# weihaoysgs/ssvio

Hardware: AMD Instinct MI355X
Metric: stereo frames/s (ORB extract + row-band match + triangulate + one local BA per frame) on 1241x376 (higher is better)
Workload: dtype u8 (front-end) + f64 (BA)

## Files before the change

include/ssx_test_hooks.h:

```cpp
#ifndef SSX_TEST_HOOKS_H
#define SSX_TEST_HOOKS_H
#include "ssx.h"

#ifdef __cplusplus
extern "C" {
#endif

SSX_API int32_t ssx_ba_window_selftest(uint32_t seed, int32_t steps);
SSX_API int32_t ssx_ba_window_debug_rewrites(const ssx_ba_window* win);

SSX_API int64_t ssx_debug_kernel_dynamic_lds(const char* kernel);
SSX_API void ssx_debug_set_dense_slabs(int32_t mode);

SSX_API void ssx_debug_set_trial_finish(int32_t mode);

SSX_API double ssx_ba_debug_prepare_seconds(const ssx_ba_problem* prob, int32_t reps);

SSX_API int32_t ssx_ba_debug_upload_format(const ssx_ba_problem* prob);

SSX_API uint64_t ssx_ba_debug_prepare_digest(const ssx_ba_problem* prob, int32_t threads);

typedef struct ssx_orb_plan_info {
  int32_t status, n_buffers;
  uint64_t digest[3];
  uint64_t arena_bytes, buf_off[32], buf_bytes[32];
  int32_t nlevels, out_cap;
  int32_t lvl_rows[8], lvl_cols[8], feat[8], lvl_cell0[9], gauss_tile0[9];
  char error[256];
} ssx_orb_plan_info;
SSX_API ssx_status ssx_orb_debug_plan(int32_t rows, int32_t cols, int32_t images, const ssx_orb_params* prm, int32_t has_mask,
                                      int32_t detect_only, int32_t unchecked, ssx_orb_plan_info* out);


SSX_API ssx_status ssx_ba_linearize(ssx_ctx* ctx, const ssx_ba_problem* prob, double huber_delta, int32_t jac_mode,
                            double* Hpp, double* bp, double* Hll, double* bl, double* Hpl, double* err,
                            double* chi2);

SSX_API ssx_status ssx_orb_stage_level(ssx_ctx* ctx, int32_t image, int32_t level, int32_t blurred,
                                       uint8_t* out, int32_t out_cap, int32_t* rows, int32_t* cols);
SSX_API ssx_status ssx_orb_stage_candidates(ssx_ctx* ctx, int32_t image, int32_t level, int32_t cap,
                                            ssx_keypoint* out, int32_t* n);

SSX_API ssx_status ssx_orb_debug_octree(ssx_ctx* ctx, int32_t rows, int32_t cols, int32_t images, const ssx_orb_params* prm,
                                        int32_t detect_only, int32_t n, const int32_t* image, const int32_t* level, const int32_t* x,
                                        const int32_t* y, const int32_t* response, int32_t* lvl_ncand, int32_t* sel_count,
                                        uint32_t* sel, int32_t* status);

SSX_API ssx_status ssx_lk_stage_level(ssx_ctx* ctx, int32_t which, int32_t level, uint8_t* out, int32_t out_cap,
                                      int32_t* rows, int32_t* cols);
SSX_API ssx_status ssx_lk_stage_deriv(ssx_ctx* ctx, int32_t level, int16_t* out, int32_t out_cap, int32_t* rows,
                                      int32_t* cols);

enum { SSX_LK_STAGED = 0, SSX_LK_ARENA = 1, SSX_LK_EACH = 2, SSX_LK_IN_PLACE = 3 };
enum { SSX_LK_K_PYRAMID = 0, SSX_LK_K_PAD_LEVEL0 = 1, SSX_LK_K_PYR_DOWN = 2, SSX_LK_K_SCHARR = 3, SSX_LK_K_TRACK = 4 };
enum { SSX_LK_SPANS = 7, SSX_LK_MAX_LAUNCHES = 32, SSX_LK_MAX_INFO_JOBS = 256 };
typedef struct ssx_lk_call_info {
  int32_t status;
  char error[256];
  int32_t levels, win, pad, rows[8], cols[8], pitch[8];
  uint64_t off[8], doff[8], pyr_bytes, deriv_words;
  int32_t fused_ok, use_fused, scharr_now, intake;
  uint64_t span_off[7], span_bytes[7], in_bytes, host_end, io_bytes, arena_bytes;
  int32_t n_launches, n_jobs;
  struct { int32_t kernel, grid[3], which, level; } launch[32];
  uint8_t slot_flags[256], job_roles[256];
} ssx_lk_call_info;
typedef struct ssx_lk_job_facts {
  int32_t slot, fresh, n, prev_stride, next_stride, reserved;
  int64_t next_off;
} ssx_lk_job_facts;
enum { SSX_LK_FACT_NEXT0_IS_HOST = 1, SSX_LK_FACT_SEVERAL_ALLOCATIONS = 2 };
SSX_API ssx_status ssx_lk_debug_plan(int32_t rows, int32_t cols, int32_t win, int32_t max_level, const int32_t* planned_key, int32_t n_jobs,
                                     const ssx_lk_job_facts* jobs, const uint8_t* slot_flags, int32_t images_on_device, int32_t call_facts,
                                     ssx_lk_call_info* out);
SSX_API ssx_status ssx_lk_debug_intake(ssx_ctx* ctx, int32_t n_jobs, const ssx_lk_job* jobs, int32_t rows, int32_t cols, const ssx_lk_params* prm,
                                       int32_t images_on_device, int32_t* intake, int32_t* arena_arithmetic);
SSX_API ssx_status ssx_lk_debug_last_call(ssx_ctx* ctx, ssx_lk_call_info* out);

SSX_API ssx_status ssx_pose_only_debug_trace(ssx_ctx* ctx, int32_t n, const ssx_pose_only_job* jobs, int32_t warmup, double* it_chi2,
                                             double* it_lambda, int32_t* it_trials, int32_t* round_rec);

enum { SSX_PO_SPANS = 6, SSX_PO_MAX_INFO_JOBS = 16, SSX_PNP_SPANS = 11 };
typedef struct ssx_po_plan_info {
  int32_t n_jobs, n_blocks, n_launches, reserved;
  struct { int32_t cls, block; uint64_t span_off[6], span_bytes[6]; } job[16];
  struct { uint64_t bytes, sent, ret_off, ret_bytes, desc_off, desc_bytes, trace_off, trace_bytes; } block[16];
  struct { int32_t cls, grid, block, first_desc; } launch[16];
} ssx_po_plan_info;
typedef struct ssx_pnp_plan_info {
  uint64_t span_off[11], span_bytes[11], bytes, sent, ret_off, ret_bytes;
  int32_t refine_cls, reserved;
} ssx_pnp_plan_info;
SSX_API ssx_status ssx_po_debug_plan(int32_t n, const int32_t* M, int32_t traced, ssx_po_plan_info* out, int32_t pnp_M, int32_t pnp_H,
                                     int32_t pnp_tap, ssx_pnp_plan_info* pnp_out);

SSX_API ssx_status ssx_pnp_debug_samples(ssx_ctx* ctx, uint32_t seed, int32_t M, int32_t H, int32_t* triples_out);
SSX_API ssx_status ssx_pnp_debug_counts(ssx_ctx* ctx, const double* K4, int32_t M, const double* xyz, const double* uv,
                                        int32_t max_iters, double reproj_px, uint32_t seed, int32_t* counts_out);
SSX_API ssx_status ssx_pnp_debug_p3p(ssx_ctx* ctx, const double* K4, int32_t n, const double* xyz, const double* uv, int32_t* valid_out,
                                     double* R_out, double* t_out, double* pose_out);

SSX_API ssx_status ssx_kfdb_debug_last_step(const ssx_kf_database* db, int32_t* launches, int32_t* synchronisations, int64_t* bytes_up,
                                            int64_t* bytes_down);
SSX_API ssx_status ssx_kfdb_debug_last_batch(ssx_ctx* ctx, int32_t* launches, int32_t* synchronisations, int64_t* bytes_up, int64_t* bytes_down);
SSX_API ssx_status ssx_kfdb_debug_bow(ssx_vocabulary* voc, const uint8_t* desc, int32_t n, int32_t cap, int32_t* ids_out, double* vals_out,
                                      int32_t* n_entries);

SSX_API ssx_status ssx_undistort_debug_last_call(ssx_ctx* ctx, int32_t* launches, int32_t* synchronisations, int64_t* bytes_up, int64_t* bytes_down);
SSX_API ssx_status ssx_undistort_plan_debug_last_call(const ssx_undistort_plan* plan, int32_t* launches, int32_t* synchronisations, int64_t* bytes_up,
                                                      int64_t* bytes_down, int32_t* copies_up, int32_t* copies_down);
SSX_API ssx_status ssx_undistort_plan_debug_map(ssx_undistort_plan* plan, int32_t map_index, uint16_t* out);
SSX_API ssx_status ssx_lens_debug_atan(ssx_ctx* ctx, int32_t n, const double* r, double* atan_out, double* sqrt_out);

SSX_API ssx_status ssx_dense_debug_last_call(ssx_ctx* ctx, int32_t* launches, int32_t* synchronisations, int64_t* bytes_up, int64_t* bytes_down,
                                             int32_t* groups);
SSX_API ssx_status ssx_dense_debug_stages(ssx_ctx* ctx, const uint8_t* left, int32_t left_stride, const uint8_t* right, int32_t right_stride,
                                          int32_t rows, int32_t cols, const ssx_dense_params* prm, int32_t direction, uint64_t* census_left,
                                          uint64_t* census_right, uint8_t* path_volume, uint16_t* sum_volume, uint8_t* right_disparity);

#ifdef __cplusplus
}
#endif
#endif
```

ssvio_amd/csrc/octree.hip:

```cpp
#include "orb_ws.hpp"

namespace ssxorb {

namespace {

typedef unsigned long long u64;
constexpr int T = OCT_THREADS;
constexpr int NW = T / 64;
constexpr unsigned NONE = 0xFFFFu;
struct Box { int16_t ulx, uly, brx, bry; };

struct Tab {
  u64* c4;
  u64* kid4;
  Box* box;
  uint32_t* key;
  uint16_t* cnt;
  uint16_t* pidx;
  uint16_t* newpos;
  uint16_t* proc;
  uint16_t* exp;
};

__device__ __forceinline__ Tab carve(uint8_t* base, int LN)
{
  Tab o;
  const size_t n = (size_t)LN;
  o.c4 = (u64*)base;
  o.kid4 = o.c4 + n;
  o.box = (Box*)(o.kid4 + n);
  o.key = (uint32_t*)(o.box + 2 * n);
  o.cnt = (uint16_t*)(o.key + n);
  o.pidx = o.cnt + 2 * n;
  o.newpos = o.pidx + n;
  o.proc = o.newpos + n;
  o.exp = o.proc + n;
  return o;
}
static_assert(OCT_NODE_BYTES == 8 + 8 + 16 + 4 + 4 + 2 + 2 + 2 + 4, "Tab layout and OCT_NODE_BYTES disagree");

__device__ __forceinline__ u64 block_scan(u64 v, u64 (*s_w)[NW], int& par, u64& total)
{
  const int lane = threadIdx.x & 63, wave = threadIdx.x >> 6;
  u64 inc = v;
#pragma unroll
  for (int o = 1; o < 64; o <<= 1) {
    const u64 up = __shfl_up(inc, o);
    if (lane >= o) inc += up;
  }
  if (lane == 63) s_w[par][wave] = inc;
  __syncthreads();
  u64 before = 0, tot = 0;
#pragma unroll
  for (int w = 0; w < NW; ++w) {
    const u64 x = s_w[par][w];
    tot += x;
    if (w < wave) before += x;
  }
  par ^= 1;
  total = tot;
  return before + (inc - v);
}

__device__ __forceinline__ int quadrant(int x, int y, const Box& n)
{
  const int mx = n.ulx + ((n.brx - n.ulx + 1) >> 1);
  const int my = n.uly + ((n.bry - n.uly + 1) >> 1);
  return (x < mx) ? ((y < my) ? 0 : 2) : ((y < my) ? 1 : 3);
}

__device__ __forceinline__ unsigned f16(u64 v, int q) { return (unsigned)((v >> (16 * q)) & 0xFFFFu); }
__device__ __forceinline__ int pk_x(uint32_t p) { return (int)(p & 0xFFF); }
__device__ __forceinline__ int pk_y(uint32_t p) { return (int)((p >> 12) & 0xFFF); }
__device__ __forceinline__ uint32_t pk_r(uint32_t p) { return p >> 24; }
__device__ __forceinline__ int nonzero4(u64 c) { return (f16(c, 0) > 0) + (f16(c, 1) > 0) + (f16(c, 2) > 0) + (f16(c, 3) > 0); }
__device__ __forceinline__ int above1_4(u64 c) { return (f16(c, 0) > 1) + (f16(c, 1) > 1) + (f16(c, 2) > 1) + (f16(c, 3) > 1); }

template <bool GLOBAL_TAB, bool GLOBAL_KEYS>
__global__ __launch_bounds__(OCT_THREADS) void k_octree(OrbDev d)
{
  extern __shared__ __attribute__((aligned(16))) uint8_t smem[];
  __shared__ u64 s_w[2][NW];
  __shared__ int s_root[64], s_rootpos[64];
  __shared__ int s_i[2];
  const int img = blockIdx.x, level = blockIdx.y, t = threadIdx.x;
  const int lane = t & 63;
  if (d.detect_only && level > 0) return;
  const int il = img * d.nlevels + level;
  const int LN = d.oct_ln;
  Tab tb;
  uint32_t* s_cellpos;
  const int CAP = d.oct_cand_cap;
  const int SLOTS = oct_key_slots(CAP);
  uint8_t* scratch = d.oct + (size_t)il * d.oct_stride;
  if constexpr (GLOBAL_TAB) {
    tb = carve(scratch + (GLOBAL_KEYS ? 6 * (size_t)SLOTS : 0), LN);
    s_cellpos = reinterpret_cast<uint32_t*>(smem);
  } else {
    tb = carve(smem, LN);
    s_cellpos = reinterpret_cast<uint32_t*>(smem + (((size_t)OCT_NODE_BYTES * LN + 15) & ~size_t(15)));
  }
  uint32_t* s_kpk;
  uint16_t* s_kn;
  if constexpr (GLOBAL_KEYS) {
    s_kpk = reinterpret_cast<uint32_t*>(scratch);
    s_kn = reinterpret_cast<uint16_t*>(s_kpk + SLOTS);
  } else {
    s_kpk = s_cellpos + ((d.oct_max_cells + 1 + 3) & ~3);
    s_kn = reinterpret_cast<uint16_t*>(s_kpk + SLOTS);
  }
  const int N = d.feat[level];
  const int cell0 = d.lvl_cell0[level], cell1 = d.lvl_cell0[level + 1];
  const int ncell = cell1 - cell0;
  const int* ccount = d.cell_count + (size_t)img * d.n_cells + cell0;
  const uint32_t* __restrict__ ccand = d.cell_cand + ((size_t)img * d.n_cells + cell0) * CELL_CAP;
  int par = 0;

  int M;
  {
    const int chunk = (ncell + T - 1) / T;
    const int lo = min(t * chunk, ncell), hi = min(lo + chunk, ncell);
    u64 mine = 0;
    for (int c = lo; c < hi; ++c) mine += (u64)ccount[c];
    u64 total;
    uint32_t pos = (uint32_t)block_scan(mine, s_w, par, total);
    for (int c = lo; c < hi; ++c) { s_cellpos[c] = pos; pos += (uint32_t)ccount[c]; }
    if (t == 0) {
      s_cellpos[ncell] = (uint32_t)total;
      d.lvl_ncand[il] = (int)total;
      if (total > (u64)CAP) atomicOr(&d.status[img], 1);
    }
    M = (int)min(total, (u64)CAP);
    if (t < 64) s_root[t] = 0;
  }
  __syncthreads();
  int* sel_count = d.sel_count + il;
  uint32_t* sel = d.sel + (size_t)il * SEL_CAP;
  if (M == 0) { if (t == 0) *sel_count = 0; return; }

  const int minX = EDGE_THRESHOLD - 3, minY = minX;
  const int maxX = d.lvl_cols[level] - EDGE_THRESHOLD + 3, maxY = d.lvl_rows[level] - EDGE_THRESHOLD + 3;
  const int nIni = (int)roundf((float)(maxX - minX) / (float)(maxY - minY));
  static_assert(OCT_MAX_ROOTS == 64, "the roots are placed by one wave, in s_root[64]");
  if (nIni < 1 || nIni > OCT_MAX_ROOTS) { if (t == 0) *sel_count = 0; return; }
  const float hX = (float)(maxX - minX) / (float)nIni;
  const int kchunk = (M + T - 1) / T;
  const int p0 = min(t * kchunk, M);
  const int nk = min(kchunk, M - p0);
  {
    int c = 0, off = 0, cend = 0;
    if (nk > 0) {
      int lo = 0, hi = ncell;
      while (hi - lo > 1) { const int mid = (lo + hi) >> 1; if (s_cellpos[mid] <= (uint32_t)p0) lo = mid; else hi = mid; }
      c = lo;
      off = p0 - (int)s_cellpos[c];
      cend = (int)(s_cellpos[c + 1] - s_cellpos[c]);
    }
    int run_root = -1, run_n = 0;
    for (int k = 0; k < nk; ++k) {
      while (off >= cend) { ++c; off = 0; cend = (int)(s_cellpos[c + 1] - s_cellpos[c]); }
      const uint32_t v = ccand[(size_t)c * CELL_CAP + off];
      ++off;
      s_kpk[k * T + t] = v;
      const int rt = (int)((float)pk_x(v) / hX);
      const int root = rt >= nIni ? nIni - 1 : rt;
      s_kn[k * T + t] = (uint16_t)root;
      if (root != run_root) {
        if (run_n > 0) atomicAdd(&s_root[run_root], run_n);
        run_root = root; run_n = 0;
      }
      ++run_n;
    }
    if (run_n > 0) atomicAdd(&s_root[run_root], run_n);
  }
  __syncthreads();
  if (t < 64) {
    const int c = t < nIni ? s_root[t] : 0;
    const u64 bal = __ballot(c > 0);
    const int pos = __popcll(bal & ((1ull << lane) - 1ull));
    s_rootpos[t] = pos;
    if (c > 0) {
      Box b;
      b.ulx = (int16_t)(int)(hX * (float)t); b.uly = 0;
      b.brx = (int16_t)(int)(hX * (float)(t + 1)); b.bry = (int16_t)(maxY - minY);
      tb.box[pos] = b;
      tb.cnt[pos] = (uint16_t)c;
    }
    if (t == 0) s_i[0] = __popcll(bal);
  }
  __syncthreads();
  int nNodes = s_i[0];
  for (int k = 0; k < nk; ++k) s_kn[k * T + t] = (uint16_t)s_rootpos[s_kn[k * T + t]];

  int cur = 0, ecur = 0, nExp = 0, phase = 1, guard = 0;
  bool finish = false;
  while (!finish && ++guard < 256) {
    const Box* bx = tb.box + cur * LN;
    const uint16_t* ct = tb.cnt + cur * LN;
    Box* nbx = tb.box + (cur ^ 1) * LN;
    uint16_t* nct = tb.cnt + (cur ^ 1) * LN;
    const uint16_t* exp_cur = tb.exp + ecur * LN;
    uint16_t* exp_nxt = tb.exp + (ecur ^ 1) * LN;
    const int prevSize = nNodes;
    const int nchunk = (nNodes + T - 1) / T;
    const int nlo = min(t * nchunk, nNodes), nhi = min(nlo + nchunk, nNodes);
    int m = 0;
    if (phase == 1) {
      u64 mine = 0;
      for (int j = nlo; j < nhi; ++j) mine += ct[j] > 1;
      u64 total;
      uint32_t pos = (uint32_t)block_scan(mine, s_w, par, total);
      for (int j = nlo; j < nhi; ++j) {
        if (ct[j] > 1) { tb.proc[pos] = (uint16_t)j; tb.pidx[j] = (uint16_t)pos; tb.c4[pos] = 0; ++pos; }
        else tb.pidx[j] = (uint16_t)NONE;
      }
      m = (int)total;
    } else {
      const int nExp4 = (nExp + 3) & ~3;
      for (int i = t; i < nExp4; i += T) tb.key[i] = i < nExp ? (((uint32_t)ct[exp_cur[i]] << 16) | (uint32_t)i) : 0u;
      for (int j = nlo; j < nhi; ++j) tb.pidx[j] = (uint16_t)NONE;
      __syncthreads();
      for (int i = t; i < nExp; i += T) {
        const uint32_t ki = tb.key[i];
        int rank = 0;
#pragma unroll 4
        for (int l = 0; l < nExp4; l += 4) {
          const uint4 kk = *reinterpret_cast<const uint4*>(&tb.key[l]);
          rank += (kk.x > ki) + (kk.y > ki) + (kk.z > ki) + (kk.w > ki);
        }
        const int j = exp_cur[i];
        tb.proc[rank] = (uint16_t)j; tb.pidx[j] = (uint16_t)rank; tb.c4[rank] = 0;
      }
      m = nExp;
    }
    __syncthreads();
    {
      unsigned run_pi = NONE;
      u64 run_c = 0;
      for (int k = 0; k < nk; ++k) {
        const int j = s_kn[k * T + t] & 0x3FFF;
        const uint32_t v = s_kpk[k * T + t];
        const unsigned pi = tb.pidx[j];
        const int q = quadrant(pk_x(v), pk_y(v), bx[j]);
        s_kn[k * T + t] = (uint16_t)(j | (q << 14));
        if (pi != run_pi) {
          if (run_pi != NONE) atomicAdd(&tb.c4[run_pi], run_c);
          run_pi = pi; run_c = 0;
        }
        run_c += 1ull << (16 * q);
      }
      if (run_pi != NONE) atomicAdd(&tb.c4[run_pi], run_c);
    }
    __syncthreads();
    int pchunk = (m + T - 1) / T;
    int plo = min(t * pchunk, m), phi = min(plo + pchunk, m);
    if (phase == 2) {
      u64 mine = 0;
      for (int i = plo; i < phi; ++i) mine += (u64)(nonzero4(tb.c4[i]) - 1);
      u64 total;
      uint32_t run = (uint32_t)block_scan(mine, s_w, par, total);
      if (t == 0) s_i[0] = m;
      __syncthreads();
      for (int i = plo; i < phi; ++i) {
        const uint32_t before = run;
        run += (uint32_t)(nonzero4(tb.c4[i]) - 1);
        if ((int)(nNodes + before) < N && (int)(nNodes + run) >= N) s_i[0] = i + 1;
      }
      __syncthreads();
      const int mt = s_i[0];
      for (int i = mt + t; i < m; i += T) tb.pidx[tb.proc[i]] = (uint16_t)NONE;
      m = mt;
      __syncthreads();
      pchunk = (m + T - 1) / T;
      plo = min(t * pchunk, m); phi = min(plo + pchunk, m);
    }
    uint32_t Tchild, EXtot, Kkeep;
    uint32_t run_cc, run_ex, run_k;
    {
      u64 mine = 0;
      for (int i = plo; i < phi; ++i) {
        const u64 c = tb.c4[i];
        mine += (u64)nonzero4(c) | ((u64)above1_4(c) << 16);
      }
      for (int j = nlo; j < nhi; ++j) mine += (u64)(tb.pidx[j] == NONE) << 32;
      u64 total;
      const u64 run = block_scan(mine, s_w, par, total);
      Tchild = (uint32_t)(total & 0xFFFFu); EXtot = (uint32_t)((total >> 16) & 0xFFFFu); Kkeep = (uint32_t)((total >> 32) & 0xFFFFu);
      run_cc = (uint32_t)(run & 0xFFFFu); run_ex = (uint32_t)((run >> 16) & 0xFFFFu); run_k = (uint32_t)((run >> 32) & 0xFFFFu);
    }
    const int nNew = (int)(Tchild + Kkeep);
    if (nNew > LN) {
      if (t == 0) atomicOr(&d.status[img], 2);
      break;
    }
    for (int i = plo; i < phi; ++i) {
      const int j = tb.proc[i];
      const Box x = bx[j];
      const u64 c = tb.c4[i];
      const int cc = nonzero4(c);
      const int mx = x.ulx + ((x.brx - x.ulx + 1) >> 1);
      const int my = x.uly + ((x.bry - x.uly + 1) >> 1);
      const int first = (int)Tchild - (int)run_cc - cc;
      int above = cc;
      u64 kid = 0;
      for (int q = 0; q < 4; ++q) {
        const int n = (int)f16(c, q);
        if (n == 0) continue;
        --above;
        const int id = first + above;
        Box ch;
        ch.ulx = (int16_t)((q & 1) ? mx : x.ulx); ch.brx = (int16_t)((q & 1) ? x.brx : mx);
        ch.uly = (int16_t)((q & 2) ? my : x.uly); ch.bry = (int16_t)((q & 2) ? x.bry : my);
        nbx[id] = ch;
        nct[id] = (uint16_t)n;
        kid |= (u64)id << (16 * q);
        if (n > 1) exp_nxt[run_ex++] = (uint16_t)id;
      }
      tb.kid4[i] = kid;
      run_cc += (uint32_t)cc;
    }
    for (int j = nlo; j < nhi; ++j)
      if (tb.pidx[j] == NONE) {
        const uint32_t np = Tchild + run_k++;
        tb.newpos[j] = (uint16_t)np;
        nbx[np] = bx[j];
        nct[np] = ct[j];
      }
    __syncthreads();
    for (int k = 0; k < nk; ++k) {
      const int kn = s_kn[k * T + t];
      const int j = kn & 0x3FFF, q = kn >> 14;
      const unsigned pi = tb.pidx[j];
      s_kn[k * T + t] = (pi != NONE) ? (uint16_t)f16(tb.kid4[pi], q) : tb.newpos[j];
    }
    __syncthreads();
    cur ^= 1;
    ecur ^= 1;
    nNodes = nNew;
    nExp = (int)EXtot;
    if (nNodes >= N || nNodes == prevSize) finish = true;
    else if (phase == 1 && nNodes + 3 * nExp > N) phase = 2;
  }
  __syncthreads();
  {
    uint32_t* best = tb.key;
    for (int j = t; j < nNodes; j += T) best[j] = 0;
    __syncthreads();
    {
      int run_j = -1;
      uint32_t run_best = 0;
      for (int k = 0; k < nk; ++k) {
        const int j = s_kn[k * T + t] & 0x3FFF;
        const uint32_t v = (pk_r(s_kpk[k * T + t]) << 16) | (uint32_t)(0xFFFF - (p0 + k));
        if (j != run_j) {
          if (run_j >= 0) atomicMax(&best[run_j], run_best);
          run_j = j; run_best = 0;
        }
        run_best = max(run_best, v);
      }
      if (run_j >= 0) atomicMax(&best[run_j], run_best);
    }
    __syncthreads();
    const int nOut = min(nNodes, SEL_CAP);
    for (int k = 0; k < nk; ++k) {
      const int j = s_kn[k * T + t] & 0x3FFF;
      const uint32_t c = s_kpk[k * T + t];
      if (j < nOut && best[j] == ((pk_r(c) << 16) | (uint32_t)(0xFFFF - (p0 + k)))) sel[j] = c;
    }
    if (t == 0) {
      *sel_count = nOut;
      if (nNodes > SEL_CAP) atomicOr(&d.status[img], 4);
    }
  }
}

}

void launch_octree(const OrbDev& o, hipStream_t s)
{
  const dim3 grid(o.I, o.detect_only ? 1 : o.nlevels);
  const size_t tab = o.oct_global_tab ? 0 : (((size_t)OCT_NODE_BYTES * o.oct_ln + 15) & ~size_t(15));
  const size_t lds = tab + 4 * (size_t)((o.oct_max_cells + 1 + 3) & ~3) + (o.oct_global_keys ? 0 : 6 * (size_t)oct_key_slots(o.oct_cand_cap));
  void (*kern)(OrbDev) = o.oct_global_tab ? (o.oct_global_keys ? k_octree<true, true> : k_octree<true, false>)
                                          : (o.oct_global_keys ? k_octree<false, true> : k_octree<false, false>);
  if (lds > 48 * 1024)
    (void)hipFuncSetAttribute(reinterpret_cast<const void*>(kern), hipFuncAttributeMaxDynamicSharedMemorySize, (int)lds);
  hipLaunchKernelGGL(kern, grid, dim3(OCT_THREADS), lds, s, o);
}

}
```

Measured before the change: 18350.

## Dispatch octree kernel by candidate-count size class with smaller blocks

After: 18160. -1.1%, worse.

```diff
diff --git a/include/ssx_test_hooks.h b/include/ssx_test_hooks.h
--- a/include/ssx_test_hooks.h
+++ b/include/ssx_test_hooks.h
@@ -45,6 +45,9 @@
                                         int32_t detect_only, int32_t n, const int32_t* image, const int32_t* level, const int32_t* x,
                                         const int32_t* y, const int32_t* response, int32_t* lvl_ncand, int32_t* sel_count,
                                         uint32_t* sel, int32_t* status);
+
+SSX_API void ssx_debug_set_octree_classes(int32_t mode);
+SSX_API int32_t ssx_orb_debug_octree_class(int32_t cls, int32_t* threads, int32_t* max_candidates);
 
 SSX_API ssx_status ssx_lk_stage_level(ssx_ctx* ctx, int32_t which, int32_t level, uint8_t* out, int32_t out_cap,
                                       int32_t* rows, int32_t* cols);
diff --git a/ssvio_amd/csrc/octree.hip b/ssvio_amd/csrc/octree.hip
--- a/ssvio_amd/csrc/octree.hip
+++ b/ssvio_amd/csrc/octree.hip
@@ -1,3 +1,7 @@
+#include <atomic>
+#include <cstdlib>
+
+#include "../../include/ssx_test_hooks.h"
 #include "orb_ws.hpp"
 
 namespace ssxorb {
@@ -5,8 +9,6 @@
 namespace {
 
 typedef unsigned long long u64;
-constexpr int T = OCT_THREADS;
-constexpr int NW = T / 64;
 constexpr unsigned NONE = 0xFFFFu;
 struct Box { int16_t ulx, uly, brx, bry; };
 
@@ -39,6 +41,7 @@
 }
 static_assert(OCT_NODE_BYTES == 8 + 8 + 16 + 4 + 4 + 2 + 2 + 2 + 4, "Tab layout and OCT_NODE_BYTES disagree");
 
+template <int NW>
 __device__ __forceinline__ u64 block_scan(u64 v, u64 (*s_w)[NW], int& par, u64& total)
 {
   const int lane = threadIdx.x & 63, wave = threadIdx.x >> 6;
@@ -76,9 +79,11 @@
 __device__ __forceinline__ int nonzero4(u64 c) { return (f16(c, 0) > 0) + (f16(c, 1) > 0) + (f16(c, 2) > 0) + (f16(c, 3) > 0); }
 __device__ __forceinline__ int above1_4(u64 c) { return (f16(c, 0) > 1) + (f16(c, 1) > 1) + (f16(c, 2) > 1) + (f16(c, 3) > 1); }
 
-template <bool GLOBAL_TAB, bool GLOBAL_KEYS>
-__global__ __launch_bounds__(OCT_THREADS) void k_octree(OrbDev d)
-{
+template <bool GLOBAL_TAB, bool GLOBAL_KEYS, int T, int KEYS>
+__global__ __launch_bounds__(T) void k_octree(OrbDev d, int m_lo)
+{
+  static_assert(T % 64 == 0 && T >= 64 && T <= OCT_THREADS && KEYS % T == 0 && (KEYS == 0 ? T == OCT_THREADS : !GLOBAL_KEYS), "size class");
+  constexpr int NW = T / 64;
   extern __shared__ __attribute__((aligned(16))) uint8_t smem[];
   __shared__ u64 s_w[2][NW];
   __shared__ int s_root[64], s_rootpos[64];
@@ -87,11 +92,15 @@
   const int lane = t & 63;
   if (d.detect_only && level > 0) return;
   const int il = img * d.nlevels + level;
+  if (m_lo >= 0) {
+    const int m = d.lvl_ncand[il];
+    if (m <= m_lo || (KEYS > 0 && m > KEYS)) return;
+  }
   const int LN = d.oct_ln;
   Tab tb;
   uint32_t* s_cellpos;
   const int CAP = d.oct_cand_cap;
-  const int SLOTS = oct_key_slots(CAP);
+  const int SLOTS = KEYS > 0 ? KEYS : oct_key_slots(CAP);
   uint8_t* scratch = d.oct + (size_t)il * d.oct_stride;
   if constexpr (GLOBAL_TAB) {
     tb = carve(scratch + (GLOBAL_KEYS ? 6 * (size_t)SLOTS : 0), LN);
@@ -127,10 +136,12 @@
     for (int c = lo; c < hi; ++c) { s_cellpos[c] = pos; pos += (uint32_t)ccount[c]; }
     if (t == 0) {
       s_cellpos[ncell] = (uint32_t)total;
-      d.lvl_ncand[il] = (int)total;
-      if (total > (u64)CAP) atomicOr(&d.status[img], 1);
-    }
-    M = (int)min(total, (u64)CAP);
+      if (m_lo < 0) {
+        d.lvl_ncand[il] = (int)total;
+        if (total > (u64)CAP) atomicOr(&d.status[img], 1);
+      }
+    }
+    M = (int)min(total, (u64)(KEYS > 0 ? min(CAP, KEYS) : CAP));
     if (t < 64) s_root[t] = 0;
   }
   __syncthreads();
@@ -157,10 +168,7 @@
       cend = (int)(s_cellpos[c + 1] - s_cellpos[c]);
     }
     int run_root = -1, run_n = 0;
-    for (int k = 0; k < nk; ++k) {
-      while (off >= cend) { ++c; off = 0; cend = (int)(s_cellpos[c + 1] - s_cellpos[c]); }
-      const uint32_t v = ccand[(size_t)c * CELL_CAP + off];
-      ++off;
+    auto place = [&](int k, uint32_t v) {
       s_kpk[k * T + t] = v;
       const int rt = (int)((float)pk_x(v) / hX);
       const int root = rt >= nIni ? nIni - 1 : rt;
@@ -170,6 +178,21 @@
         run_root = root; run_n = 0;
       }
       ++run_n;
+    };
+    auto next = [&]() {
+      while (off >= cend) { ++c; off = 0; cend = (int)(s_cellpos[c + 1] - s_cellpos[c]); }
+      return ccand[(size_t)c * CELL_CAP + off++];
+    };
+    if constexpr (!GLOBAL_KEYS) {
+      static_assert(CAND_CAP % OCT_THREADS == 0, "whole key slots per thread");
+      constexpr int KPT = (KEYS > 0 ? KEYS : CAND_CAP) / T;
+      uint32_t kv[KPT];
+#pragma unroll
+      for (int k = 0; k < KPT; ++k) kv[k] = k < nk ? next() : 0u;
+#pragma unroll
+      for (int k = 0; k < KPT; ++k) if (k < nk) place(k, kv[k]);
+    } else {
+      for (int k = 0; k < nk; ++k) place(k, next());
     }
     if (run_n > 0) atomicAdd(&s_root[run_root], run_n);
   }
@@ -374,18 +397,79 @@
   }
 }
 
-}
-
-void launch_octree(const OrbDev& o, hipStream_t s)
-{
-  const dim3 grid(o.I, o.detect_only ? 1 : o.nlevels);
+__global__ __launch_bounds__(64) void k_octree_count(OrbDev d)
+{
+  const int img = blockIdx.x, level = blockIdx.y, lane = threadIdx.x;
+  const int il = img * d.nlevels + level;
+  const int cell0 = d.lvl_cell0[level], ncell = d.lvl_cell0[level + 1] - cell0;
+  const int* ccount = d.cell_count + (size_t)img * d.n_cells + cell0;
+  int n = 0;
+  for (int c = lane; c < ncell; c += 64) n += ccount[c];
+#pragma unroll
+  for (int o = 32; o > 0; o >>= 1) n += __shfl_xor(n, o);
+  if (lane == 0) {
+    d.lvl_ncand[il] = n;
+    if (n > d.oct_cand_cap) atomicOr(&d.status[img], 1);
+    if (n == 0) d.sel_count[il] = 0;
+  }
+}
+
+std::atomic<int> g_classes{-1};
+inline int classes_mode()
+{
+  int m = g_classes.load(std::memory_order_relaxed);
+  if (m < 0) {
+    const char* e = getenv("SSX_OCT_CLASSES");
+    m = (e && e[0] == '0') ? 0 : 1;
+    g_classes.store(m, std::memory_order_relaxed);
+  }
+  return m;
+}
+
+size_t oct_lds(const OrbDev& o, int key_slots)
+{
   const size_t tab = o.oct_global_tab ? 0 : (((size_t)OCT_NODE_BYTES * o.oct_ln + 15) & ~size_t(15));
-  const size_t lds = tab + 4 * (size_t)((o.oct_max_cells + 1 + 3) & ~3) + (o.oct_global_keys ? 0 : 6 * (size_t)oct_key_slots(o.oct_cand_cap));
-  void (*kern)(OrbDev) = o.oct_global_tab ? (o.oct_global_keys ? k_octree<true, true> : k_octree<true, false>)
-                                          : (o.oct_global_keys ? k_octree<false, true> : k_octree<false, false>);
+  return tab + 4 * (size_t)((o.oct_max_cells + 1 + 3) & ~3) + 6 * (size_t)key_slots;
+}
+
+void launch_one(void (*kern)(OrbDev, int), const dim3& grid, int threads, size_t lds, hipStream_t s, const OrbDev& o, int m_lo)
+{
   if (lds > 48 * 1024)
     (void)hipFuncSetAttribute(reinterpret_cast<const void*>(kern), hipFuncAttributeMaxDynamicSharedMemorySize, (int)lds);
-  hipLaunchKernelGGL(kern, grid, dim3(OCT_THREADS), lds, s, o);
-}
-
-}
+  hipLaunchKernelGGL(kern, grid, dim3(threads), lds, s, o, m_lo);
+}
+
+}
+
+constexpr int OCT_CLASS_THREADS[3] = {256, 512, OCT_THREADS};
+constexpr int OCT_CLASS_KEYS[3] = {4096, 8192, CAND_CAP};
+
+void launch_octree(const OrbDev& o, hipStream_t s)
+{
+  const dim3 grid(o.I, o.detect_only ? 1 : o.nlevels);
+  if (classes_mode() && !o.oct_global_tab && !o.oct_global_keys) {
+    hipLaunchKernelGGL(k_octree_count, grid, dim3(64), 0, s, o);
+    launch_one(k_octree<false, false, OCT_THREADS, 0>, grid, OCT_THREADS, oct_lds(o, oct_key_slots(o.oct_cand_cap)), s, o, OCT_CLASS_KEYS[1]);
+    launch_one(k_octree<false, false, OCT_CLASS_THREADS[1], OCT_CLASS_KEYS[1]>, grid, OCT_CLASS_THREADS[1], oct_lds(o, OCT_CLASS_KEYS[1]), s, o, OCT_CLASS_KEYS[0]);
+    launch_one(k_octree<false, false, OCT_CLASS_THREADS[0], OCT_CLASS_KEYS[0]>, grid, OCT_CLASS_THREADS[0], oct_lds(o, OCT_CLASS_KEYS[0]), s, o, 0);
+    return;
+  }
+  void (*kern)(OrbDev, int) = o.oct_global_tab ? (o.oct_global_keys ? k_octree<true, true, OCT_THREADS, 0> : k_octree<true, false, OCT_THREADS, 0>)
+                                               : (o.oct_global_keys ? k_octree<false, true, OCT_THREADS, 0> : k_octree<false, false, OCT_THREADS, 0>);
+  launch_one(kern, grid, OCT_THREADS, oct_lds(o, o.oct_global_keys ? 0 : oct_key_slots(o.oct_cand_cap)), s, o, -1);
+}
+
+#ifndef SSX_NO_TEST_HOOKS
+extern "C" {
+void ssx_debug_set_octree_classes(int32_t mode) { g_classes.store(mode < 0 ? -1 : (mode ? 1 : 0)); }
+int32_t ssx_orb_debug_octree_class(int32_t cls, int32_t* threads, int32_t* max_candidates)
+{
+  if (cls < 0 || cls > 2) return -1;
+  if (threads) *threads = OCT_CLASS_THREADS[cls];
+  if (max_candidates) *max_candidates = OCT_CLASS_KEYS[cls];
+  return 0;
+}
+}
+#endif
+
+}
```
